# OpenMined/PIR

Hardware: AMD Instinct MI355X
Metric: PIR queries/sec (ms/query in ms_per_step), N=4096 DB=2^20 x 288B d=2 (higher is better)
Workload: dtype u64

## Files before the change

### pir_amd/csrc/ctx.hip

```cpp
#include <hip/hip_runtime.h>
#include <ctype.h>
#include <stdint.h>
#include <stdio.h>
#include <stdlib.h>
#include <string.h>

#include <algorithm>
#include <atomic>
#include <functional>
#include <map>
#include <mutex>
#include <string>
#include <vector>

#include "../../include/pirgpu.h"
#include "device_params.h"
#include "host_math.h"
#include "kernels.h"
#include "wire.h"

using namespace pirgpu;

namespace {

// ... 158 lines not shown
  uint64_t pt_words = 0;
  BatchSet sets[kBatchSets];
  BatchSet& bs();
  uint32_t n_active = 1;
  uint32_t upper_blocks = 512;
  uint32_t upper_blocks_batch = 64;
  uint32_t scan_wgs_batch = 128;
  bool in_batch = false;
  uint32_t scan_nsplit = 1, scan_cps = 0, scan_rows = 0, scan_cols = 0;
  uint32_t scan_rpt = 4, scan_block = 256;
  bool scan_limb = false;
  uint32_t mq_nq = 4, mq_rows = 1;
  bool mq_single = true;
  uint32_t mq_single_rows = 4;
  bool mq_single_limb = false;
  uint64_t scan_npt = 0;
  bool mfma_on = false;
  MfmaGeom mg{};
  uint32_t mfma_nq = kMaxMfmaQueries;
  bool mfma_single = true;
  bool scan_f64_fold = false;
  bool scan_f64_fold_batch = false;
  bool split_upper = false;
  uint64_t split_upper_words = (3ull << 30) / 8;
  bool loop_transforms = true;
  uint32_t loop_min_sources = 1024;
  uint32_t fuse_mac_nodes = 128;
  bool fuse_mac_combine = true;
  bool fuse_last_level = true;
  bool last_level_ntt = true;
  bool tree40 = true;
  bool c0_ntt = false;
  bool c0_ntt_split = false;
  bool want_sel_f64 = true;
  bool sel_f64 = false;
  bool pack40 = false;
  int pack_bytes = 5;
  uint8_t* d_dbp = nullptr;
  bool packed_valid = false;
  bool staging_released = false;
  std::vector<BatchLane> lanes;
  uint64_t groups_run = 0;
  hipStream_t head_stream = nullptr;
  uint32_t head_levels = 5;
  uint32_t head_mode = 1;
  hipEvent_t ev_head_tail = nullptr;
  hipStream_t copy_stream = nullptr;
  hipEvent_t ev_fetch[2] = {nullptr, nullptr};
  hipEvent_t ev_fork = nullptr;
  hipEvent_t ev_main_join = nullptr;

  bool prof = false;
  std::vector<hipEvent_t> bscan_ev;
  uint32_t bscan_n = 0, bscan_wgs = 0, bscan_nq = 0;
  static constexpr int kMaxProfRuns = 256;
  std::vector<hipEvent_t> ev;
  int prof_runs = 0;
  int prof_cur = -1;
  float timings[6]{};

  std::map<std::string, int64_t> opts;
  std::string err;
  uint64_t gen = 0;
  std::recursive_mutex mu;
  uint64_t zero_pts = 0;
  uint64_t remote_zero_pts = 0;
// ... 220 lines not shown
  }
  c->scan_npt = shard_pts;
  {
    auto env_u32 = [c](const char* name, uint32_t dflt) {
      return (uint32_t)option(c, name + 7, dflt);
    };
    c->scan_limb = true;
    for (uint32_t j = 0; j < k; ++j) c->scan_limb = c->scan_limb && (c->hp.mod[j].q >> 50) == 0;
    if (!env_u32("PIRGPU_SCAN_LIMB", 1)) c->scan_limb = false;
    c->mq_nq = 4;
    c->mq_rows = 1;
    c->mq_single = env_u32("PIRGPU_SCAN_MQ_SINGLE", 1) != 0;
    c->mq_single_rows = 4;
    c->mq_single_limb = false;
    c->scan_rpt = env_u32("PIRGPU_SCAN_ROWS", 4);
    c->scan_block = env_u32("PIRGPU_SCAN_BLOCK", 256);
    const uint32_t xblocks = (k * N / 2 + c->scan_block - 1) / c->scan_block;
    const uint32_t yblocks = (c->scan_rows + c->scan_rpt - 1) / c->scan_rpt;
    uint64_t have = (uint64_t)xblocks * std::max<uint32_t>(yblocks, 1) * c->scan_block / 256;
    uint32_t want = have >= 512 ? 1 : (uint32_t)ceil_div(1024, std::max<uint64_t>(have, 1));
    want = env_u32("PIRGPU_SCAN_NSPLIT", want);
    want = std::max<uint32_t>(1, std::min<uint32_t>(want, std::max<uint32_t>(c->scan_cols, 1)));
    c->scan_cps = (uint32_t)ceil_div(std::max<uint32_t>(c->scan_cols, 1), want);
    c->scan_nsplit = (uint32_t)ceil_div(std::max<uint32_t>(c->scan_cols, 1), c->scan_cps);
    c->fuse_last_level = env_u32("PIRGPU_FUSE_LAST", 1) != 0;
    c->fuse_mac_combine = env_u32("PIRGPU_FUSE_MAC_COMBINE", 1) != 0;
    c->last_level_ntt = env_u32("PIRGPU_LAST_NTT", 1) != 0;
    {
      const uint32_t v = env_u32("PIRGPU_C0_NTT", 0);
      c->c0_ntt = v != 0;
      c->c0_ntt_split = v >= 2;
    }
    c->want_sel_f64 = env_u32("PIRGPU_SEL_F64", 1) != 0;
    c->tree40 = env_u32("PIRGPU_TREE40", 1) != 0;
    c->fuse_mac_nodes = 128;
    c->head_levels = std::min<uint32_t>(env_u32("PIRGPU_HEAD_LEVELS", c->head_levels), 8);
    c->head_mode = std::min<uint32_t>(env_u32("PIRGPU_HEAD_MODE", c->head_mode), 2);
    c->split_upper = env_u32("PIRGPU_SPLIT_UPPER", c->logN >= 14 ? 1 : 0) != 0 && c->mode != kNttInt;
    c->split_upper_words = (uint64_t)env_u32("PIRGPU_SPLIT_UPPER_MB", 3072) * (1ull << 20) / 8;
    c->loop_transforms = env_u32("PIRGPU_LOOP_TRANSFORMS", 1) != 0 && c->mode != kNttInt;
    c->pack40 = env_u32("PIRGPU_PACK40", 1) != 0;
    {
      uint32_t bits = 0;
      for (uint32_t j = 0; j <= k; ++j) bits = std::max<uint32_t>(bits, 64 - (uint32_t)__builtin_clzll(c->hp.mod[j].q));
      const int need = bits <= 39 ? 5 : (bits <= 47 ? 6 : (bits <= 55 ? 7 : 8));
      int want = (int)env_u32("PIRGPU_PACK_BYTES", (uint32_t)need);
      if (want < need) want = need;
      if (c->mode == kNttInt && want != 5) want = 8;
      if (want > 7) c->pack40 = false;
      c->pack_bytes = c->pack40 ? want : 5;
      if (c->pack40 && c->pack_bytes == 7 && c->logN >= 14 && !env_u32("PIRGPU_TREE40_WIDE", 0)) c->tree40 = false;
      const NttOps* ops = ntt_ops_for(N, c->pack_bytes);
      if (ops != c->ops) {
        c->ops = ops;
        HIP_TRY(c->ops->configure(c->mode));
      }
    }
    bool wide_given = false;
    const int64_t wide = option(c, "SCAN_MFMA_WIDE", 0, &wide_given);
    c->mg = mfma_geometry(c->hp, c->scan_rows, c->scan_cols, wide_given ? (int)(wide != 0) : -1,
                          env_u32("PIRGPU_SCAN_MFMA_TOP4", 1) != 0);
    c->mfma_on = env_u32("PIRGPU_SCAN_MFMA", 1) != 0 && d >= 2 && c->mg.L != 0 && c->scan_rows >= 8 && shard_pts > 0;
    if (c->slot_sharded && (!c->mfma_on || c->mg.nchunks != 1 || c->nslots % c->mg.NW))
      throw Fail{PIRGPU_INVALID_ARGUMENT, "a slot shard needs the int8-MFMA scan in one column chunk (d = 2, >= 8 rows, "
                                          "moduli below 2^55, at most 28 column groups)"};
    c->mfma_nq = std::max<uint32_t>(1, std::min<uint32_t>(env_u32("PIRGPU_SCAN_MFMA_NQ", kMaxMfmaQueries),
// ... 140 lines not shown
  HIP_TRY(hipStreamSynchronize(st));
  c->gperm[g] = buf;
  return buf;
}

struct TreeState {
  uint64_t* cur = nullptr;
  bool cur40 = false;
  bool c0ntt = false;
};

uint64_t* expand_core(pirgpu_ctx* c, hipStream_t st, uint64_t* res_a, uint64_t* res_b, uint64_t* dig, uint64_t* prod,
                      uint32_t n, uint32_t B, const MfmaPtrs* sel_dst = nullptr, bool sel_f64 = false,
                      const uint32_t* ksets = nullptr, uint32_t j_begin = 0, uint32_t j_end = UINT32_MAX,
                      const TreeState* from = nullptr, TreeState* to = nullptr,
                      const std::function<void()>& after_first = nullptr) {
  const uint32_t N = c->N, k = c->k;
  if (n > N) throw Fail{PIRGPU_INVALID_ARGUMENT, "Cannot expand more items from a CT than poly modulus degree"};
  const uint32_t logm = hm::ceil_log2(n);
  const bool fuse_last = sel_dst && c->mode != kNttInt && c->fuse_last_level;
  if (sel_f64 && !(fuse_last && c->last_level_ntt && n >= 2)) throw Fail{PIRGPU_INTERNAL, "double-form selectors need the NTT-domain last level"};
  uint64_t *cur = res_a, *nxt = res_b;
  bool cur40 = false;
  bool c0ntt = false;
  if (from) {
    cur = from->cur;
    cur40 = from->cur40;
    c0ntt = from->c0ntt;
    nxt = res_a;
  }
  const uint32_t j_stop = std::min(j_end, logm);
  const bool c0_path = c->c0_ntt && fuse_last && c->last_level_ntt && c->mode != kNttInt && c->fuse_mac_combine;
  const uint32_t fuse_from = B > 1 ? std::max<uint32_t>(c->fuse_mac_nodes / 2, 1) : c->fuse_mac_nodes;
  auto level_fused = [&](uint32_t j) {
    return c->mode != kNttInt && c->fuse_mac_combine && ((1u << j) * B) >= fuse_from && !(fuse_last && j + 1 == logm);
  };
  for (uint32_t j = j_begin; j < j_stop; ++j) {
    auto level_done = [&]() {
      if (from && j == j_begin) {
        nxt = res_b;
        if (after_first) after_first();
      }
    };
    const uint32_t g = (N >> j) + 1;
    const KeyPtrs key = keys_for(c, g, ksets, B);
    const uint32_t nodes = (1u << j) * B;
    const bool last_ntt = fuse_last && j + 1 == logm && c->last_level_ntt;
    const bool c0_in_digit = last_ntt && !c0ntt && ks_digit_takes_c0(nodes);
    if (cur40 && !(last_ntt ? (c0ntt || c0_in_digit) : true)) throw Fail{PIRGPU_INTERNAL, "5-byte tree reached a level that cannot read it"};
    if (c0_path && !c0ntt && level_fused(j) && !cur40 && !(from && j == j_begin)) {
      HIP_TRY(c->ops->tree_c0_fwd(st, c->mode, c->dp, k, cur, nodes));
      c0ntt = true;
    }
    HIP_TRY(c->ops->ks_digit(st, c->mode, c->dp, k, cur, g, nodes, dig, c->pack40, c0_in_digit ? prod : nullptr, cur40,
                             c->loop_transforms && (uint64_t)nodes * k >= c->loop_min_sources));
    if (level_fused(j)) {
      const uint32_t next_nodes = nodes * 2;
      const bool next_last = j + 2 == logm;
      const bool next_reads40 = next_last ? (fuse_last && c->last_level_ntt && (c0ntt || ks_digit_takes_c0(next_nodes)))
                                          : (next_nodes >= fuse_from);
      const bool out40 = c->tree40 && c->pack40 && j + 1 < logm && next_reads40 && (1u << j) < (N >> ntt_log_ept((int)c->logN));
      HIP_TRY(c->ops->ks_mac_intt(st, c->mode, c->dp, k, dig, key, nodes, prod, c->pack40, k, 1));
      HIP_TRY(c->ops->ks_mac_combine(st, c->mode, c->dp, k, dig, key, prod, cur, g, nodes, 1u << j, nxt, c->pack40, cur40,
                                     out40, c0ntt ? xpow_table(c, st, 1u << j) : nullptr,
                                     c0ntt ? galois_perm_table(c, st, g) : nullptr, c->c0_ntt_split));
      cur40 = out40;
      std::swap(cur, nxt);
      level_done();
      continue;
    }
    if (cur40 && !last_ntt) throw Fail{PIRGPU_INTERNAL, "5-byte tree reached an unfused level"};
    if (c0ntt && !last_ntt) throw Fail{PIRGPU_INTERNAL, "NTT-form c0 reached an unfused level"};
    if (fuse_last && j + 1 == logm && c->last_level_ntt) {
      const uint64_t* X = xpow_table(c, st, 1u << j);
      HIP_TRY(c->ops->ks_mac_intt(st, c->mode, c->dp, k, dig, key, nodes, prod, c->pack40, k, 1));
      HIP_TRY(c->ops->ks_last_ntt(st, c->mode, c->dp, k, cur, dig, key, prod, X, g, galois_inverse(g, N), 1u << j, n, B,
                                  *sel_dst, nodes, c->pack40, sel_f64, c0_in_digit, c0ntt ? (cur40 ? 2 : 1) : 0,
                                  galois_perm_table(c, st, g)));
      return nullptr;
    }
    HIP_TRY(c->ops->ks_mac_intt(st, c->mode, c->dp, k, dig, key, nodes, prod, c->pack40, 0, k + 1));
    if (fuse_last && j + 1 == logm) {
      HIP_TRY(c->ops->ks_last_level(st, c->mode, c->dp, k, cur, prod, g, 1u << j, n, B, *sel_dst, nodes, c->pack40));
      return nullptr;
    }
// ... 394 lines not shown
  delete c;
}

const char* pirgpu_last_error(const pirgpu_ctx* c) {
  if (!c) return "null context";
  if (t_last_error_ctx == c && t_last_error_gen == c->gen)
    return t_last_error.c_str();
  return c->err.c_str();
}

void pirgpu_set_error(pirgpu_ctx* c, const char* message) { (void)fail(c, 0, message ? message : ""); }

void pirgpu_request_lock(pirgpu_ctx* c) {
  if (c) c->mu.lock();
}
void pirgpu_request_unlock(pirgpu_ctx* c) {
  if (c) c->mu.unlock();
}

int pirgpu_set_transparent_policy(pirgpu_ctx* c, int allow) {
  return guarded(c, [&]() -> int {
    c->allow_transparent = allow != 0;
    return PIRGPU_OK;
  });
}

static const struct { const char* name; bool early; } kOptions[] = {
    {"UPPER_BLOCKS", true}, {"UPPER_BLOCKS_BATCH", true}, {"SCAN_MFMA_WGS_BATCH", false}, {"SCAN_LIMB", true},
    {"SCAN_MQ_SINGLE", true}, {"SCAN_ROWS", true}, {"SCAN_BLOCK", true}, {"SCAN_NSPLIT", true},
    {"FUSE_LAST", true}, {"FUSE_MAC_COMBINE", true}, {"LAST_NTT", true}, {"C0_NTT", true}, {"SEL_F64", true}, {"TREE40", true},
    {"SPLIT_UPPER", true}, {"SPLIT_UPPER_MB", true}, {"PACK40", true}, {"PACK_BYTES", true}, {"TREE40_WIDE", true},
    {"SCAN_MFMA", true}, {"SCAN_MFMA_WIDE", true}, {"SCAN_MFMA_TOP4", true}, {"SCAN_MFMA_NQ", true}, {"SCAN_MFMA_SINGLE", true},
    {"HEAD_LEVELS", true}, {"HEAD_MODE", true}, {"SCAN_F64_FOLD", true}, {"SCAN_F64_FOLD_BATCH", true}, {"LOOP_TRANSFORMS", true},
    {"SLOTS_SCAN_WGS", false}, {"SLOTS_GATHER_NTT", false}, {"SLOTS_SCAN_BLK_MAJOR", false},
};

int pirgpu_set_option(pirgpu_ctx* c, const char* name, int64_t value) {
  return guarded(c, [&]() -> int {
    if (!name) return fail(c, PIRGPU_INVALID_ARGUMENT, "null option name");
    std::string up(name);
    for (char& ch : up) ch = (char)toupper((unsigned char)ch);
    for (const auto& o : kOptions) {
      if (up != o.name) continue;
      if (o.early && c->ws_ready)
        return fail(c, PIRGPU_FAILED_PRECONDITION, "option " + up + " shapes the workspace: set it before the context is first used");
      c->opts[up] = value;
      if (up == "SCAN_MFMA_WGS_BATCH") c->scan_wgs_batch = (uint32_t)std::max<int64_t>(0, value);
      return PIRGPU_OK;
    }
    return fail(c, PIRGPU_INVALID_ARGUMENT, "unknown option " + up);
  });
}

int pirgpu_get_option(pirgpu_ctx* c, const char* name, int64_t* value) {
  return guarded(c, [&]() -> int {
    if (!name || !value) return fail(c, PIRGPU_INVALID_ARGUMENT, "null argument");
    std::string up(name);
    for (char& ch : up) ch = (char)toupper((unsigned char)ch);
    for (const auto& o : kOptions)
      if (up == o.name) {
        bool present = false;
        *value = option(c, o.name, -1, &present);
        return PIRGPU_OK;
      }
    return fail(c, PIRGPU_INVALID_ARGUMENT, "unknown option " + up);
  });
}
// ... 1713 lines not shown
```

### pir_amd/csrc/kernels.h

```cpp
#pragma once
#include <hip/hip_runtime.h>
#include <stdint.h>

#include "device_params.h"

namespace pirgpu {

constexpr int kMaxScanChunks = 16;
constexpr int kMaxMfmaQueries = 8;
constexpr int kMaxScanGroups = 16;
constexpr int kMaxSlices = 16;

constexpr uint32_t kKsWideLevel = 256;
inline bool ks_digit_takes_c0(uint32_t nodes) { return nodes >= kKsWideLevel && nodes % 8 == 0; }

struct MfmaPtrs {
  const void* p[kMaxMfmaQueries];
};

struct ScanGroups {
  uint32_t n;
  const uint8_t* sel[kMaxScanGroups];
  uint64_t* out[kMaxScanGroups];
  uint8_t nq[kMaxScanGroups];
// ... 24 lines not shown
  hipError_t (*ks_digit)(hipStream_t st, int mode, const DevParams* P, uint32_t k, const uint64_t* res_in,
                         uint32_t galois_elt, uint32_t nodes, uint64_t* dig, bool pack40, uint64_t* c0_out, bool tree40,
                         bool loop_targets);
  hipError_t (*ks_mac_intt)(hipStream_t st, int mode, const DevParams* P, uint32_t k, const uint64_t* dig,
                            const KeyPtrs& key, uint32_t nodes, uint64_t* prod, bool pack40, uint32_t I_base,
                            uint32_t I_count);
  hipError_t (*upper_fused)(hipStream_t st, int mode, const DevParams* P, uint32_t k, uint32_t enc_count,
                            const uint64_t* src, const MfmaPtrs& svq, uint64_t* part, uint32_t n_rows,
                            uint32_t n_dim, uint32_t n_children_total, uint32_t sv_first, uint32_t C,
                            uint32_t chunk_len, uint32_t n_chunks, uint32_t n_queries, uint64_t src_qstride,
                            uint64_t part_qstride, bool sel_f64);
  hipError_t (*ks_last_level)(hipStream_t st, int mode, const DevParams* P, uint32_t k, const uint64_t* tree,
                              const uint64_t* prod, uint32_t galois_elt, uint32_t shift_pow, uint32_t n_items,
                              uint32_t B, const MfmaPtrs& dst, uint32_t tree_cts, bool pack40);
  hipError_t (*upper_ntt)(hipStream_t st, int mode, const DevParams* P, uint32_t k, uint32_t enc_count,
                          const uint64_t* src, uint64_t* scratch, uint32_t n_rows, uint32_t n_dim,
                          uint32_t n_children_total, uint32_t C, uint32_t b0, uint32_t blk, uint32_t n_queries,
                          uint64_t src_qstride, bool loop_source);
  hipError_t (*ks_mac_combine)(hipStream_t st, int mode, const DevParams* P, uint32_t k, const uint64_t* dig,
                               const KeyPtrs& key, const uint64_t* prod, const uint64_t* tree_in, uint32_t galois_elt,
                               uint32_t nodes, uint32_t shift_pow, uint64_t* tree_out, bool pack40, bool tin40,
                               bool tout40, const uint64_t* xpow_c0ntt,
                               const uint16_t* perm,
                               bool c0_split);
  hipError_t (*ks_last_ntt)(hipStream_t st, int mode, const DevParams* P, uint32_t k, const uint64_t* tree,
                            const uint64_t* dig, const KeyPtrs& key, uint64_t* prod, const uint64_t* xpow,
                            uint32_t galois_elt, uint32_t galois_inv, uint32_t shift_pow, uint32_t n_items, uint32_t B,
                            const MfmaPtrs& dst, uint32_t nodes, bool pack40, bool out_f64, bool c0_done, int c0_tree,
                            const uint16_t* perm);
  hipError_t (*ntt_inv_gather)(hipStream_t st, int mode, const DevParams* P, uint32_t k, const uint64_t* src,
                               uint64_t* dst, const SliceMap& map, uint32_t RC, uint32_t nq, uint32_t nq_total,
                               uint32_t q0);
  hipError_t (*tree_c0_fwd)(hipStream_t st, int mode, const DevParams* P, uint32_t k, uint64_t* tree, uint32_t cts);
};

const NttOps* ntt_ops_for(uint32_t N, int pack_bytes = 5);

hipError_t launch_ntt_reorder(hipStream_t st, uint32_t N, const uint64_t* in, uint64_t* out, uint64_t n_polys,
                              bool to_device, bool as_f64);
hipError_t launch_pack40x4(hipStream_t st, const uint64_t* in, uint32_t* out, uint64_t words);
hipError_t launch_unpack40x4(hipStream_t st, const uint32_t* in, uint64_t* out, uint64_t words);
hipError_t launch_ks_combine(hipStream_t st, const DevParams* P, int mode, uint32_t N, uint32_t k,
                             const uint64_t* res_in, const uint64_t* prod, uint32_t galois_inv, uint32_t nodes,
                             uint32_t shift_pow, bool expand_step, uint32_t hi_limit, bool pack40, uint64_t* res_out,
                             int pack_bytes = 5);
hipError_t launch_tree_convert(hipStream_t st, const DevParams* P, int mode, const uint64_t* in, uint64_t* out,
                               uint64_t words, bool to_tree, uint64_t chunk_words = 0, uint64_t in_stride = 0);
hipError_t launch_monomial_shift(hipStream_t st, const DevParams* P, uint32_t N, uint32_t k, const uint64_t* in,
                                 uint32_t shift, uint64_t count, uint64_t* out);
hipError_t launch_scan(hipStream_t st, const DevParams* P, uint32_t N, uint32_t k, const uint64_t* db,
                       const uint64_t* sv, uint64_t* out, uint32_t rows, uint32_t cols, uint64_t num_pt,
                       uint32_t nsplit, uint32_t cols_per_split, uint32_t rows_per_thread, uint32_t block,
                       bool limb);
hipError_t launch_scan_mq(hipStream_t st, const DevParams* P, uint32_t N, uint32_t k, const uint64_t* db,
                          const uint64_t* const* sv, uint64_t* const* out, uint32_t nq, uint32_t rows,
                          uint32_t cols, uint32_t rows_per_wave, bool limb);
hipError_t launch_reduce_splits(hipStream_t st, const DevParams* P, const uint64_t* part, uint32_t nsplit,
                                uint64_t words, uint64_t* out, uint32_t n_queries = 1, uint64_t part_qstride = 0,
                                uint64_t out_qstride = 0);


hipError_t launch_upper_mac(hipStream_t st, const DevParams* P, const uint64_t* scratch, const MfmaPtrs& svq,
                            uint64_t* acc, uint64_t* out, uint32_t n_queries, uint32_t n_rows, uint32_t C,
                            uint32_t enc_count, uint32_t k, uint32_t N, uint32_t sv_first, uint32_t b0, uint32_t blk,
                            uint32_t n_dim, bool first, bool last, uint64_t acc_qstride, uint64_t out_qstride);

// ... 32 lines not shown
```

### pir_amd/csrc/ntt_kernels.hip

```cpp
#include <hip/hip_runtime.h>
#include <stdint.h>
#include <stdlib.h>

#include "device_params.h"
#include "kernels.h"
#include "ntt_core.h"

#ifndef PIRGPU_LOGN
#error "compile with -DPIRGPU_LOGN=<11..14>"
#endif

#ifndef PIRGPU_PACK_BYTES
#define PIRGPU_PACK_BYTES 5
#endif
#define PIRGPU_CAT2(a, b) a##b
#define PIRGPU_CAT(a, b) PIRGPU_CAT2(a, b)
#if PIRGPU_PACK_BYTES == 5
#define PIRGPU_OPS_NAME PIRGPU_CAT(ntt_ops_, PIRGPU_LOGN)
#define PIRGPU_DEG_NS PIRGPU_CAT(deg, PIRGPU_LOGN)
#else
#define PIRGPU_OPS_NAME PIRGPU_CAT(PIRGPU_CAT(ntt_ops_, PIRGPU_LOGN), PIRGPU_CAT(_p, PIRGPU_PACK_BYTES))
#define PIRGPU_DEG_NS PIRGPU_CAT(PIRGPU_CAT(deg, PIRGPU_LOGN), PIRGPU_CAT(p, PIRGPU_PACK_BYTES))
#endif

// ... 683 lines not shown
    for (int e = 0; e < EPT; ++e) tlo[e * NT + tid_e] = t[e];
  }
  uint32_t tid_x = tid_e;
  asm volatile("" : "+v"(tid_x) : : "memory");
#pragma unroll
  for (int e = 0; e < EPT; ++e) t[e] = f64_mulmod(f64_norm(v[e] - x[e], m), X[e * NT + tid_x], m);
  if constexpr (TOUT40) {
    store40f(reinterpret_cast<uint8_t*>(tree_out_raw) + phi * kPoly40, tid_x, t, magic);
  } else {
    double* thi = reinterpret_cast<double*>(tree_out_raw) + phi * N;
#pragma unroll
    for (int e = 0; e < EPT; ++e) thi[e * NT + tid_x] = t[e];
  }
}

template <int MODE, bool P40, bool TIN40, bool TOUT40>
__global__ void __launch_bounds__(NT)
ks_c0_ntt_kernel(const DevParams* __restrict__ P, const uint64_t* __restrict__ dig_raw, KeyPtrs keys,
                 const uint64_t* __restrict__ prod, const uint64_t* __restrict__ tree_in_raw, uint32_t galois_elt,
                 uint32_t nodes, uint64_t* __restrict__ tree_out_raw, const double* __restrict__ xpow,
                 const uint16_t* __restrict__ perm) {
  static_assert(MODE != kNttInt, "fp64 flavours only");
  const uint32_t k = P->k;
  uint32_t node = blockIdx.x, j = blockIdx.y;
  if (gridDim.y == 1) {
    const uint32_t xcd = blockIdx.x & 7, t = blockIdx.x >> 3;
    j = t % k;
    node = (t / k) * 8 + xcd;
  }
  ks_combine_c0_ntt<MODE, P40, TIN40, TOUT40>(P, dig_raw, keys.p[node % keys.B], prod, tree_in_raw, xpow, perm, galois_elt, nodes,
                                              node, j, threadIdx.x, tree_out_raw);
}

template <int MODE, bool P40, bool TIN40 = false, bool TOUT40 = false, bool C0NTT = false>
__global__ void __launch_bounds__(NT) PIRGPU_MC_WAVES PIRGPU_PK_WAVES
ks_mac_combine_kernel(const DevParams* __restrict__ P, const uint64_t* __restrict__ dig_raw,
                      KeyPtrs keys, const uint64_t* __restrict__ prod,
                      const uint64_t* __restrict__ tree_in_raw, uint32_t galois_elt, uint32_t nodes, uint32_t shift_pow,
                      uint64_t* __restrict__ tree_out_raw, const double* __restrict__ xpow,
                      const uint16_t* __restrict__ perm, uint32_t comp1_only) {
  using A = Arith<MODE>;
  static_assert(MODE != kNttInt, "fp64 flavours only");
  double* sd = reinterpret_cast<double*>(smem_raw);
  const uint32_t tid = threadIdx.x, k = P->k, km = k + 1;
  uint32_t node = blockIdx.x, j = blockIdx.y, comp = blockIdx.z;
  if (gridDim.y == 1 && gridDim.z == 1) {
    const uint32_t xcd = blockIdx.x & 7, t = blockIdx.x >> 3;
    comp = comp1_only ? 1 : t & 1;
    const uint32_t u = comp1_only ? t : t >> 1;
    j = u % k;
    node = (u / k) * 8 + xcd;
  } else if (comp1_only) {
    comp = 1;
  }
  if constexpr (C0NTT) {
    if (comp == 0) {
      ks_combine_c0_ntt<MODE, P40, TIN40, TOUT40>(P, dig_raw, keys.p[node % keys.B], prod, tree_in_raw, xpow, perm, galois_elt,
                                                  nodes, node, j, tid, tree_out_raw);
      return;
    }
  }
  const typename A::Mod m = A::mod(P, j);
  double g[EPT];
  ks_mac_core<MODE, P40>(P, dig_raw, keys.p[node % keys.B], node, j, comp, tid, g);
  {
    const double pf = P->p_f, half = P->p_half_f, pinv = P->p_inv_f[j];
// ... 1 lines not shown
    [[maybe_unused]] Hi16 hs{};
    if constexpr (P40) hs = load40f_hi(reinterpret_cast<const uint8_t*>(prod) + spoly * kPoly40, tid);
#pragma unroll
    for (int e = 0; e < EPT; ++e) {
      double sp;
      if constexpr (P40) {
        sp = load40f(reinterpret_cast<const uint8_t*>(prod) + spoly * kPoly40, hs, e, tid, f64_pack_magic(pf));
      } else {
        sp = reinterpret_cast<const double*>(prod)[spoly * N + e * NT + tid];
      }
      sp = sp > half ? sp - pf : sp;
      sp = sp < -half ? sp + pf : sp;
      g[e] = f64_mulmod(g[e] - f64_norm(sp, m), pinv, m);
    }
  }
  if (!C0NTT && comp == 0) {
    const uint32_t raw0 = tid * galois_elt, rstep = (uint32_t)NT * galois_elt;
    double c0[EPT];
    tree_load<TIN40>(tree_in_raw, (size_t)node * 2 * k + j, tid, m.q, c0);
    __syncthreads();
#pragma unroll
    for (int e = 0; e < EPT; ++e) {
      const uint32_t raw = raw0 + (uint32_t)e * rstep;
      const uint64_t sign = (uint64_t)((raw << (31 - LOGN)) & 0x80000000u) << 32;
      sd[lds_idx<R_>(raw & (N - 1))] = __longlong_as_double((long long)((uint64_t)__double_as_longlong(c0[e]) ^ sign));
    }
    __syncthreads();
#pragma unroll
    for (int e = 0; e < EPT; ++e) g[e] += sd[lds_lin_base<NT, R_>(tid) + lds_lin_off<NT, R_>(e)];
  }
  const size_t opoly = (size_t)comp * k + j;
  double a[EPT];
  tree_load<TIN40>(tree_in_raw, (size_t)node * 2 * k + opoly, tid, m.q, a);
  if constexpr (TOUT40) {
    const double magic = f64_pack_magic(m.q);
    uint8_t* plo = reinterpret_cast<uint8_t*>(tree_out_raw) + ((size_t)node * 2 * k + opoly) * kPoly40;
    uint8_t* phi = reinterpret_cast<uint8_t*>(tree_out_raw) + (((size_t)node + nodes) * 2 * k + opoly) * kPoly40;
    double lo[EPT];
#pragma unroll
    for (int e = 0; e < EPT; ++e) lo[e] = f64_norm(a[e] + g[e], m);
    store40f(plo, tid, lo, magic);
    const bool borrow = tid < shift_pow;
    const uint32_t tid_d = (tid - shift_pow) & (NT - 1);
    uint32_t hb[EPT];
#pragma unroll
    for (int e = 0; e < EPT; ++e) {
      double d = f64_norm(a[e] - g[e], m);
      if (e == 0) d = borrow ? -d : d;
      uint32_t l32;
      f64_pack40(d, magic, l32, hb[e]);
      reinterpret_cast<uint32_t*>(phi)[(e * NT + tid - shift_pow) & (N - 1)] = l32;
    }
    uint32_t w[kHW];
    pack_hi_bytes(hb, w);
    uint32_t o[kHW];
#pragma unroll
    for (int q4 = 0; q4 < kHW; ++q4)
      o[q4] = borrow ? __builtin_amdgcn_alignbyte(w[(q4 + 1) % kHW], w[q4], kHB) : w[q4];
    store_hi_words(phi, tid_d, o);
  } else {
    const size_t off = opoly * N;
    double* tree_lo = reinterpret_cast<double*>(tree_out_raw) + (size_t)node * 2 * k * N + off;
    double* tree_hi = reinterpret_cast<double*>(tree_out_raw) + ((size_t)node + nodes) * 2 * k * N + off;
#pragma unroll
    for (int e = 0; e < EPT; ++e) {
      const uint32_t i = e * NT + tid;
      tree_lo[i] = f64_norm(a[e] + g[e], m);
      const double d = f64_norm(a[e] - g[e], m);
      const uint32_t sraw = i + (2 * N - shift_pow);
      tree_hi[sraw & (N - 1)] = (sraw & N) ? -d : d;
    }
  }
}

template <int MODE, bool P40>
__global__ void __launch_bounds__(NT)
ks_last_level_kernel(const DevParams* __restrict__ P, const uint64_t* __restrict__ tree_raw,
                     const uint64_t* __restrict__ prod, uint32_t galois_elt, uint32_t shift_pow, uint32_t n_items,
                     uint32_t B, MfmaPtrs dst) {
  using A = Arith<MODE>;
  static_assert(MODE != kNttInt, "fp64 flavours only");
  double* sd = reinterpret_cast<double*>(smem_raw);
  const uint32_t tid = threadIdx.x, k = P->k, km = k + 1;
  const uint32_t half_id = blockIdx.x & 1, bx = blockIdx.x >> 1;
  const uint32_t j = bx % k, comp = (bx / k) & 1, ct = bx / (2 * k);
  const uint32_t slot = ct / B, q = ct % B;
  const uint32_t out_slot = half_id ? slot + shift_pow : slot;
  if (out_slot >= n_items) return;
  const typename A::Mod m = A::mod(P, j);
  const double pf = P->p_f, half = P->p_half_f, pinv = P->p_inv_f[j];
  const double* tree = reinterpret_cast<const double*>(tree_raw) + (size_t)ct * 2 * k * N;
  double g[EPT];
  [[maybe_unused]] Hi16 hs{}, hj{};
  if constexpr (P40) {
    const uint8_t* pr = reinterpret_cast<const uint8_t*>(prod) + ((size_t)ct * 2 + comp) * km * kPoly40;
    hs = load40f_hi(pr + (size_t)k * kPoly40, tid);
    hj = load40f_hi(pr + (size_t)j * kPoly40, tid);
  }
#pragma unroll
  for (int e = 0; e < EPT; ++e) {
    [[maybe_unused]] const uint32_t i = e * NT + tid;
    double sp, dj;
    if constexpr (P40) {
// ... 524 lines not shown
    PIRGPU_SET((ks_mac_combine_kernel<MODE, true, true, true>));
    PIRGPU_SET((ks_mac_combine_kernel<MODE, false, false, false, true>));
    PIRGPU_SET((ks_mac_combine_kernel<MODE, true, false, false, true>));
    PIRGPU_SET((ks_mac_combine_kernel<MODE, true, false, true, true>));
    PIRGPU_SET((ks_mac_combine_kernel<MODE, true, true, false, true>));
    PIRGPU_SET((ks_mac_combine_kernel<MODE, true, true, true, true>));
    PIRGPU_SET(tree_c0_fwd_kernel<MODE>);
    PIRGPU_SET((ks_c0_ntt_kernel<MODE, false, false, false>));
    PIRGPU_SET((ks_c0_ntt_kernel<MODE, true, false, false>));
    PIRGPU_SET((ks_c0_ntt_kernel<MODE, true, false, true>));
    PIRGPU_SET((ks_c0_ntt_kernel<MODE, true, true, false>));
    PIRGPU_SET((ks_c0_ntt_kernel<MODE, true, true, true>));
    PIRGPU_SET((ks_digit_kernel<MODE, true, true>));
    PIRGPU_SET((ks_digit_kernel<MODE, false, false, true>));
    PIRGPU_SET((ks_digit_kernel<MODE, true, false, true>));
    PIRGPU_SET((ks_digit_kernel<MODE, true, true, true>));
    PIRGPU_SET((upper_ntt_kernel<MODE, true>));
    PIRGPU_SET((ks_last_level_kernel<MODE, false>));
    PIRGPU_SET((ks_last_level_kernel<MODE, true>));
    PIRGPU_SET((tree_c0_ntt_kernel<MODE, false>));
    PIRGPU_SET((tree_c0_ntt_kernel<MODE, true>));
    PIRGPU_SET((ks_last_ntt_kernel<MODE, false>));
    PIRGPU_SET((ks_last_ntt_kernel<MODE, true>));
    PIRGPU_SET((ks_last_ntt_kernel<MODE, false, true>));
    PIRGPU_SET((ks_last_ntt_kernel<MODE, true, true>));
    PIRGPU_SET((ks_last_ntt_kernel<MODE, false, false, 1>));
    PIRGPU_SET((ks_last_ntt_kernel<MODE, false, true, 1>));
    PIRGPU_SET((ks_last_ntt_kernel<MODE, true, false, 1>));
    PIRGPU_SET((ks_last_ntt_kernel<MODE, true, true, 1>));
    PIRGPU_SET((ks_last_ntt_kernel<MODE, true, false, 2>));
    PIRGPU_SET((ks_last_ntt_kernel<MODE, true, true, 2>));
    PIRGPU_SET((upper_fused_kernel<MODE, false, true>));
  }
#undef PIRGPU_SET
  return hipSuccess;
}

static hipError_t op_configure(int mode) {
  PIRGPU_BY_MODE(mode, return configure_mode<MODE>());
  return hipSuccess;
}

static hipError_t op_ntt_batch(hipStream_t st, int mode, const DevParams* P, uint64_t* data, uint64_t n_polys,
                               uint32_t mod_period, uint32_t mod_base, bool inverse) {
  if (inverse) {
    PIRGPU_BY_MODE(mode, hipLaunchKernelGGL((ntt_batch_kernel<MODE, true>), dim3((uint32_t)n_polys), dim3(NT),
                                            kLdsBytes, st, P, data, mod_period, mod_base));
  } else {
    PIRGPU_BY_MODE(mode, hipLaunchKernelGGL((ntt_batch_kernel<MODE, false>), dim3((uint32_t)n_polys), dim3(NT),
                                            kLdsBytes, st, P, data, mod_period, mod_base));
  }
  return hipGetLastError();
}

static hipError_t op_ntt_inv_gather(hipStream_t st, int mode, const DevParams* P, uint32_t k, const uint64_t* src,
                                    uint64_t* dst, const SliceMap& map, uint32_t RC, uint32_t nq, uint32_t nq_total,
                                    uint32_t q0) {
  if (map.n == 0 || map.n > (uint32_t)kMaxSlices || map.cut[0] != 0 || map.cut[map.n] != k * (uint32_t)N || q0 + nq > nq_total)
    return hipErrorInvalidValue;
  for (uint32_t r = 0; r <= map.n; ++r)
    if (map.cut[r] % NT) return hipErrorInvalidValue;
  PIRGPU_BY_MODE(mode, hipLaunchKernelGGL(ntt_inv_gather_kernel<MODE>, dim3(nq * RC * k), dim3(NT), kLdsBytes, st, P, src, dst,
                                          map, RC, nq_total, q0));
  return hipGetLastError();
}

// ... 242 lines not shown
    return hipErrorInvalidValue;
  return hipGetLastError();
}

static hipError_t op_upper_fused(hipStream_t st, int mode, const DevParams* P, uint32_t k, uint32_t enc_count,
                                 const uint64_t* src, const MfmaPtrs& svq, uint64_t* part, uint32_t n_rows,
                                 uint32_t n_dim, uint32_t n_children_total, uint32_t sv_first, uint32_t C,
                                 uint32_t chunk_len, uint32_t n_chunks, uint32_t n_queries, uint64_t src_qstride,
                                 uint64_t part_qstride, bool sel_f64) {
  const dim3 grid(n_queries * n_rows * C * n_chunks, enc_count, k);
#define PIRGPU_UF_ARGS P, src, svq, part, n_rows, n_dim, n_children_total, sv_first, C, chunk_len, n_chunks, src_qstride, part_qstride
  if (sel_f64 && mode == kNttInt) return hipErrorInvalidValue;
  if constexpr (kUpperLdsTw) {
    static const bool lds_tw = pirgpu_env("PIRGPU_UPPER_LDS_TW") && atoi(pirgpu_env("PIRGPU_UPPER_LDS_TW")) != 0;
    if (lds_tw && mode != kNttInt) {
      const size_t lds = kLdsBytes + (size_t)N * 8;
      if (mode == kNttF64 && sel_f64) hipLaunchKernelGGL((upper_fused_kernel<kNttF64, true, true>), grid, dim3(NT), lds, st, PIRGPU_UF_ARGS);
      else if (mode == kNttF64) hipLaunchKernelGGL((upper_fused_kernel<kNttF64, true>), grid, dim3(NT), lds, st, PIRGPU_UF_ARGS);
      else if (sel_f64) hipLaunchKernelGGL((upper_fused_kernel<kNttF64Wide, true, true>), grid, dim3(NT), lds, st, PIRGPU_UF_ARGS);
      else hipLaunchKernelGGL((upper_fused_kernel<kNttF64Wide, true>), grid, dim3(NT), lds, st, PIRGPU_UF_ARGS);
      return hipGetLastError();
    }
  }
  if (sel_f64) {
    if (mode == kNttF64) hipLaunchKernelGGL((upper_fused_kernel<kNttF64, false, true>), grid, dim3(NT), kLdsBytes, st, PIRGPU_UF_ARGS);
    else hipLaunchKernelGGL((upper_fused_kernel<kNttF64Wide, false, true>), grid, dim3(NT), kLdsBytes, st, PIRGPU_UF_ARGS);
    return hipGetLastError();
  }
  PIRGPU_BY_MODE(mode, hipLaunchKernelGGL(upper_fused_kernel<MODE>, grid, dim3(NT), kLdsBytes, st, PIRGPU_UF_ARGS));
#undef PIRGPU_UF_ARGS
  return hipGetLastError();
}

}

const NttOps* PIRGPU_OPS_NAME() {
  using namespace PIRGPU_DEG_NS;
  static const NttOps ops = {op_configure, op_ntt_batch,   op_ct_ntt_fwd_oop, op_ct_ntt_fwd_split, op_db_encode,
                             op_ks_digit,  op_ks_mac_intt, op_upper_fused,     op_ks_last_level,
                             op_upper_ntt, op_ks_mac_combine, op_ks_last_ntt, op_ntt_inv_gather, op_tree_c0_fwd};
  return &ops;
}

}
```

Measured before the change: 5556.

## Fuse key-switch digit, MAC/iNTT and tree combine into one per-node kernel

Adds a single kernel that handles one expansion-tree level per node for N=4096, k=2, 5-byte packing. It does the Galois automorphism, forward NTT of the digits, key multiply-accumulate, inverse NTT with mod-switch and the tree combine all within one workgroup of (k+1)*NT threads, keeping intermediates in LDS. This replaces three launches and their global round-trips through the digit and product buffers. The cost is heavy LDS use per block, which lowers occupancy, and more serialized work per block.

```diff
diff --git a/pir_amd/csrc/ctx.hip b/pir_amd/csrc/ctx.hip
--- a/pir_amd/csrc/ctx.hip
+++ b/pir_amd/csrc/ctx.hip
@@ -214,6 +214,7 @@
   bool tree40 = true;
   bool c0_ntt = false;
   bool c0_ntt_split = false;
+  bool ks_fused = true;
   bool want_sel_f64 = true;
   bool sel_f64 = false;
   bool pack40 = false;
@@ -500,6 +501,7 @@
       c->c0_ntt_split = v >= 2;
     }
     c->want_sel_f64 = env_u32("PIRGPU_SEL_F64", 1) != 0;
+    c->ks_fused = env_u32("PIRGPU_KS_FUSED", 1) != 0;
     c->tree40 = env_u32("PIRGPU_TREE40", 1) != 0;
     c->fuse_mac_nodes = 128;
     c->head_levels = std::min<uint32_t>(env_u32("PIRGPU_HEAD_LEVELS", c->head_levels), 8);
@@ -706,9 +708,12 @@
   const uint32_t j_stop = std::min(j_end, logm);
   const bool c0_path = c->c0_ntt && fuse_last && c->last_level_ntt && c->mode != kNttInt && c->fuse_mac_combine;
   const uint32_t fuse_from = B > 1 ? std::max<uint32_t>(c->fuse_mac_nodes / 2, 1) : c->fuse_mac_nodes;
+  const bool fused_kernel = c->ks_fused && c->ops->ks_fused && c->mode == kNttF64 && k == 2 && c->pack40 &&
+                            c->pack_bytes == 5 && !c0_path;
   auto level_fused = [&](uint32_t j) {
     return c->mode != kNttInt && c->fuse_mac_combine && ((1u << j) * B) >= fuse_from && !(fuse_last && j + 1 == logm);
   };
+  auto uses_fused_kernel = [&](uint32_t j) { return fused_kernel && B > 1 && level_fused(j); };
   for (uint32_t j = j_begin; j < j_stop; ++j) {
     auto level_done = [&]() {
       if (from && j == j_begin) {
@@ -725,6 +730,17 @@
     if (c0_path && !c0ntt && level_fused(j) && !cur40 && !(from && j == j_begin)) {
       HIP_TRY(c->ops->tree_c0_fwd(st, c->mode, c->dp, k, cur, nodes));
       c0ntt = true;
+    }
+    if (uses_fused_kernel(j)) {
+      const bool next_last = j + 2 == logm;
+      const bool next_reads40 = next_last ? (fuse_last && c->last_level_ntt && ks_digit_takes_c0(nodes * 2))
+                                          : level_fused(j + 1);
+      const bool out40 = c->tree40 && c->pack40 && j + 1 < logm && next_reads40 && (1u << j) < (N >> ntt_log_ept((int)c->logN));
+      HIP_TRY(c->ops->ks_fused(st, c->mode, c->dp, k, key, cur, g, nodes, 1u << j, nxt, cur40, out40));
+      cur40 = out40;
+      std::swap(cur, nxt);
+      level_done();
+      continue;
     }
     HIP_TRY(c->ops->ks_digit(st, c->mode, c->dp, k, cur, g, nodes, dig, c->pack40, c0_in_digit ? prod : nullptr, cur40,
                              c->loop_transforms && (uint64_t)nodes * k >= c->loop_min_sources));
@@ -1185,7 +1201,7 @@
     {"SPLIT_UPPER", true}, {"SPLIT_UPPER_MB", true}, {"PACK40", true}, {"PACK_BYTES", true}, {"TREE40_WIDE", true},
     {"SCAN_MFMA", true}, {"SCAN_MFMA_WIDE", true}, {"SCAN_MFMA_TOP4", true}, {"SCAN_MFMA_NQ", true}, {"SCAN_MFMA_SINGLE", true},
     {"HEAD_LEVELS", true}, {"HEAD_MODE", true}, {"SCAN_F64_FOLD", true}, {"SCAN_F64_FOLD_BATCH", true}, {"LOOP_TRANSFORMS", true},
-    {"SLOTS_SCAN_WGS", false}, {"SLOTS_GATHER_NTT", false}, {"SLOTS_SCAN_BLK_MAJOR", false},
+    {"KS_FUSED", true}, {"SLOTS_SCAN_WGS", false}, {"SLOTS_GATHER_NTT", false}, {"SLOTS_SCAN_BLK_MAJOR", false},
 };
 
 int pirgpu_set_option(pirgpu_ctx* c, const char* name, int64_t value) {
diff --git a/pir_amd/csrc/kernels.h b/pir_amd/csrc/kernels.h
--- a/pir_amd/csrc/kernels.h
+++ b/pir_amd/csrc/kernels.h
@@ -80,6 +80,9 @@
                                uint64_t* dst, const SliceMap& map, uint32_t RC, uint32_t nq, uint32_t nq_total,
                                uint32_t q0);
   hipError_t (*tree_c0_fwd)(hipStream_t st, int mode, const DevParams* P, uint32_t k, uint64_t* tree, uint32_t cts);
+  hipError_t (*ks_fused)(hipStream_t st, int mode, const DevParams* P, uint32_t k, const KeyPtrs& key,
+                         const uint64_t* tree_in, uint32_t galois_elt, uint32_t nodes, uint32_t shift_pow,
+                         uint64_t* tree_out, bool tin40, bool tout40);
 };
 
 const NttOps* ntt_ops_for(uint32_t N, int pack_bytes = 5);
diff --git a/pir_amd/csrc/ntt_kernels.hip b/pir_amd/csrc/ntt_kernels.hip
--- a/pir_amd/csrc/ntt_kernels.hip
+++ b/pir_amd/csrc/ntt_kernels.hip
@@ -739,6 +739,51 @@
                                               node, j, threadIdx.x, tree_out_raw);
 }
 
+template <bool TOUT40>
+__device__ __forceinline__ void ks_tree_store(uint64_t* __restrict__ tree_out_raw, uint32_t node, uint32_t nodes, uint32_t k,
+                                              size_t opoly, uint32_t shift_pow, const double (&a)[EPT],
+                                              const double (&g)[EPT], const F64Mod& m, uint32_t tid) {
+  if constexpr (TOUT40) {
+    const double magic = f64_pack_magic(m.q);
+    uint8_t* plo = reinterpret_cast<uint8_t*>(tree_out_raw) + ((size_t)node * 2 * k + opoly) * kPoly40;
+    uint8_t* phi = reinterpret_cast<uint8_t*>(tree_out_raw) + (((size_t)node + nodes) * 2 * k + opoly) * kPoly40;
+    double lo[EPT];
+#pragma unroll
+    for (int e = 0; e < EPT; ++e) lo[e] = f64_norm(a[e] + g[e], m);
+    store40f(plo, tid, lo, magic);
+    const bool borrow = tid < shift_pow;
+    const uint32_t tid_d = (tid - shift_pow) & (NT - 1);
+    uint32_t hb[EPT];
+#pragma unroll
+    for (int e = 0; e < EPT; ++e) {
+      double d = f64_norm(a[e] - g[e], m);
+      if (e == 0) d = borrow ? -d : d;
+      uint32_t l32;
+      f64_pack40(d, magic, l32, hb[e]);
+      reinterpret_cast<uint32_t*>(phi)[(e * NT + tid - shift_pow) & (N - 1)] = l32;
+    }
+    uint32_t w[kHW];
+    pack_hi_bytes(hb, w);
+    uint32_t o[kHW];
+#pragma unroll
+    for (int q4 = 0; q4 < kHW; ++q4)
+      o[q4] = borrow ? __builtin_amdgcn_alignbyte(w[(q4 + 1) % kHW], w[q4], kHB) : w[q4];
+    store_hi_words(phi, tid_d, o);
+  } else {
+    const size_t off = opoly * N;
+    double* tree_lo = reinterpret_cast<double*>(tree_out_raw) + (size_t)node * 2 * k * N + off;
+    double* tree_hi = reinterpret_cast<double*>(tree_out_raw) + ((size_t)node + nodes) * 2 * k * N + off;
+#pragma unroll
+    for (int e = 0; e < EPT; ++e) {
+      const uint32_t i = e * NT + tid;
+      tree_lo[i] = f64_norm(a[e] + g[e], m);
+      const double d = f64_norm(a[e] - g[e], m);
+      const uint32_t sraw = i + (2 * N - shift_pow);
+      tree_hi[sraw & (N - 1)] = (sraw & N) ? -d : d;
+    }
+  }
+}
+
 template <int MODE, bool P40, bool TIN40 = false, bool TOUT40 = false, bool C0NTT = false>
 __global__ void __launch_bounds__(NT) PIRGPU_MC_WAVES PIRGPU_PK_WAVES
 ks_mac_combine_kernel(const DevParams* __restrict__ P, const uint64_t* __restrict__ dig_raw,
@@ -806,43 +851,140 @@
   const size_t opoly = (size_t)comp * k + j;
   double a[EPT];
   tree_load<TIN40>(tree_in_raw, (size_t)node * 2 * k + opoly, tid, m.q, a);
-  if constexpr (TOUT40) {
-    const double magic = f64_pack_magic(m.q);
-    uint8_t* plo = reinterpret_cast<uint8_t*>(tree_out_raw) + ((size_t)node * 2 * k + opoly) * kPoly40;
-    uint8_t* phi = reinterpret_cast<uint8_t*>(tree_out_raw) + (((size_t)node + nodes) * 2 * k + opoly) * kPoly40;
-    double lo[EPT];
-#pragma unroll
-    for (int e = 0; e < EPT; ++e) lo[e] = f64_norm(a[e] + g[e], m);
-    store40f(plo, tid, lo, magic);
-    const bool borrow = tid < shift_pow;
-    const uint32_t tid_d = (tid - shift_pow) & (NT - 1);
-    uint32_t hb[EPT];
+  ks_tree_store<TOUT40>(tree_out_raw, node, nodes, k, opoly, shift_pow, a, g, m, tid);
+}
+
+constexpr bool kFusedLevel = LOGN == 12 && kPB == 5;
+constexpr uint32_t kFusedK = 2;
+constexpr int kFusedNT = (int)(kFusedK + 1) * NT;
+constexpr size_t kFusedStash = (size_t)(kFusedK + 1) * Plan<LOGN>::LDS_WORDS * 8;
+constexpr size_t kFusedLdsBytes = kFusedStash + (size_t)(kFusedK + 1) * N * 4;
+
+template <bool TIN40, bool TOUT40>
+__global__ void __launch_bounds__(kFusedNT)
+ks_fused_kernel(const DevParams* __restrict__ P, KeyPtrs keys, const uint64_t* __restrict__ tree_in_raw,
+                uint32_t galois_elt, uint32_t nodes, uint32_t shift_pow, uint64_t* __restrict__ tree_out_raw) {
+  using A = Arith<kNttF64>;
+  constexpr uint32_t k = kFusedK, km = k + 1;
+  const uint32_t I = __builtin_amdgcn_readfirstlane(threadIdx.x / NT), tid = threadIdx.x % NT;
+  const bool special = I == k;
+  double* sd = reinterpret_cast<double*>(smem_raw) + (size_t)I * Plan<LOGN>::LDS_WORDS;
+  const double* sp_lds = reinterpret_cast<const double*>(smem_raw) + (size_t)k * Plan<LOGN>::LDS_WORDS;
+  uint32_t* stash = reinterpret_cast<uint32_t*>(smem_raw + kFusedStash) + (size_t)I * N;
+  const uint32_t node = blockIdx.x;
+  const double* key = reinterpret_cast<const double*>(keys.p[node % keys.B]);
+  const typename A::Mod m = A::mod(P, I);
+  const double magic = f64_pack_magic(m.q);
+  double d0[EPT], x[EPT];
+#pragma clang loop unroll(disable)
+  for (uint32_t J = 0; J < k; ++J) {
+    uint32_t tl = tid;
+    asm volatile("" : "+v"(tl));
+    const double qJd = P->tab[J].qd;
+    const uint32_t raw0 = tl * galois_elt, rstep = (uint32_t)NT * galois_elt;
+    double c1[EPT];
+    tree_load<TIN40>(tree_in_raw, ((size_t)node * 2 + 1) * k + J, tl, qJd, c1);
+    __syncthreads();
 #pragma unroll
     for (int e = 0; e < EPT; ++e) {
-      double d = f64_norm(a[e] - g[e], m);
-      if (e == 0) d = borrow ? -d : d;
-      uint32_t l32;
-      f64_pack40(d, magic, l32, hb[e]);
-      reinterpret_cast<uint32_t*>(phi)[(e * NT + tid - shift_pow) & (N - 1)] = l32;
-    }
-    uint32_t w[kHW];
-    pack_hi_bytes(hb, w);
-    uint32_t o[kHW];
-#pragma unroll
-    for (int q4 = 0; q4 < kHW; ++q4)
-      o[q4] = borrow ? __builtin_amdgcn_alignbyte(w[(q4 + 1) % kHW], w[q4], kHB) : w[q4];
-    store_hi_words(phi, tid_d, o);
-  } else {
-    const size_t off = opoly * N;
-    double* tree_lo = reinterpret_cast<double*>(tree_out_raw) + (size_t)node * 2 * k * N + off;
-    double* tree_hi = reinterpret_cast<double*>(tree_out_raw) + ((size_t)node + nodes) * 2 * k * N + off;
-#pragma unroll
-    for (int e = 0; e < EPT; ++e) {
-      const uint32_t i = e * NT + tid;
-      tree_lo[i] = f64_norm(a[e] + g[e], m);
-      const double d = f64_norm(a[e] - g[e], m);
-      const uint32_t sraw = i + (2 * N - shift_pow);
-      tree_hi[sraw & (N - 1)] = (sraw & N) ? -d : d;
+      const uint32_t raw = raw0 + (uint32_t)e * rstep;
+      const uint64_t sign = (uint64_t)((raw << (31 - LOGN)) & 0x80000000u) << 32;
+      double v = __longlong_as_double((long long)((uint64_t)__double_as_longlong(c1[e]) ^ sign));
+      v = v < 0.0 ? v + qJd : v;
+      sd[lds_idx<R_>(raw & (N - 1))] = v;
+    }
+    __syncthreads();
+#pragma unroll
+    for (int e = 0; e < EPT; ++e) x[e] = sd[lds_lin_base<NT, R_>(tl) + lds_lin_off<NT, R_>(e)];
+    __syncthreads();
+    ntt_forward<kNttF64, LOGN, false, false>(x, sd, P, I, tl);
+    if (J == 0) {
+#pragma unroll
+      for (int e = 0; e < EPT; ++e) d0[e] = x[e];
+    }
+  }
+  Hi16 hi0;
+  {
+    uint32_t hb0[EPT];
+    uint32_t tl = tid;
+    asm volatile("" : "+v"(tl));
+    const uint64_t* key64 = reinterpret_cast<const uint64_t*>(key);
+    const __amdgpu_buffer_rsrc_t r00 = poly_rsrc(key64 + ((size_t)(0 * 2 + 0) * km + I) * N);
+    const __amdgpu_buffer_rsrc_t r01 = poly_rsrc(key64 + ((size_t)(0 * 2 + 1) * km + I) * N);
+    const __amdgpu_buffer_rsrc_t r10 = poly_rsrc(key64 + ((size_t)(1 * 2 + 0) * km + I) * N);
+    const __amdgpu_buffer_rsrc_t r11 = poly_rsrc(key64 + ((size_t)(1 * 2 + 1) * km + I) * N);
+    auto kw = [&](__amdgpu_buffer_rsrc_t r, int e) { return __longlong_as_double((long long)poly_load_u64(r, tl, e)); };
+#pragma unroll
+    for (int e4 = 0; e4 < EPT; e4 += 4) {
+#pragma unroll
+      for (int e = e4; e < e4 + 4; ++e) {
+        double s0 = 0.0, s1 = 0.0;
+        s0 += f64_mulmod(d0[e], kw(r00, e), m);
+        s1 += f64_mulmod(d0[e], kw(r01, e), m);
+        s0 += f64_mulmod(x[e], kw(r10, e), m);
+        s1 += f64_mulmod(x[e], kw(r11, e), m);
+        uint32_t lo;
+        f64_pack40(f64_norm(s0, m), magic, lo, hb0[e]);
+        stash[e * NT + tl] = lo;
+        x[e] = f64_norm(s1, m);
+      }
+      asm volatile("" : "+v"(tl) : "v"(x[e4 + 3]));
+    }
+    pack_hi_bytes(hb0, hi0.w);
+  }
+  const double pf = P->p_f, half = P->p_half_f;
+  const double pinv = special ? 0.0 : P->p_inv_f[I];
+#pragma clang loop unroll(disable)
+  for (uint32_t comp = 1; comp < 2; --comp) {
+    uint32_t tl = tid;
+    asm volatile("" : "+v"(tl));
+    if (comp == 0) {
+      __syncthreads();
+#pragma unroll
+      for (int e = 0; e < EPT; ++e) {
+        const uint32_t lo = stash[e * NT + tl];
+        x[e] = __longlong_as_double((long long)(((uint64_t)hi_word(hi0, e) << 32) | lo)) - magic;
+      }
+    }
+    ntt_inverse<kNttF64, LOGN, false, false>(x, sd, P, I, tl);
+    __syncthreads();
+    if (special) {
+#pragma unroll
+      for (int e = 0; e < EPT; ++e) sd[e * NT + tl] = x[e];
+    }
+    __syncthreads();
+    if (!special) {
+#pragma unroll
+      for (int e = 0; e < EPT; ++e) {
+        double sp = sp_lds[e * NT + tl];
+        sp = sp > half ? sp - pf : sp;
+        sp = sp < -half ? sp + pf : sp;
+        x[e] = f64_mulmod(x[e] - f64_norm(sp, m), pinv, m);
+      }
+    }
+    if (comp == 0) {
+      if (!special) {
+        const uint32_t raw0 = tl * galois_elt, rstep = (uint32_t)NT * galois_elt;
+        double c0[EPT];
+        tree_load<TIN40>(tree_in_raw, (size_t)node * 2 * k + I, tl, m.q, c0);
+#pragma unroll
+        for (int e = 0; e < EPT; ++e) {
+          const uint32_t raw = raw0 + (uint32_t)e * rstep;
+          const uint64_t sign = (uint64_t)((raw << (31 - LOGN)) & 0x80000000u) << 32;
+          sd[lds_idx<R_>(raw & (N - 1))] = __longlong_as_double((long long)((uint64_t)__double_as_longlong(c0[e]) ^ sign));
+        }
+      }
+      __syncthreads();
+      if (!special) {
+#pragma unroll
+        for (int e = 0; e < EPT; ++e) x[e] += sd[lds_lin_base<NT, R_>(tl) + lds_lin_off<NT, R_>(e)];
+      }
+    }
+    if (!special) {
+      const size_t opoly = (size_t)comp * k + I;
+      double a[EPT];
+      tree_load<TIN40>(tree_in_raw, (size_t)node * 2 * k + opoly, tl, m.q, a);
+      ks_tree_store<TOUT40>(tree_out_raw, node, nodes, k, opoly, shift_pow, a, x, m, tl);
     }
   }
 }
@@ -1433,6 +1575,11 @@
     PIRGPU_SET((ks_last_ntt_kernel<MODE, true, true, 2>));
     PIRGPU_SET((upper_fused_kernel<MODE, false, true>));
   }
+  if constexpr (MODE == kNttF64 && kFusedLevel) {
+    for (const void* f : {(const void*)ks_fused_kernel<false, false>, (const void*)ks_fused_kernel<false, true>,
+                          (const void*)ks_fused_kernel<true, false>, (const void*)ks_fused_kernel<true, true>})
+      if ((e = hipFuncSetAttribute(f, hipFuncAttributeMaxDynamicSharedMemorySize, (int)kFusedLdsBytes))) return e;
+  }
 #undef PIRGPU_SET
   return hipSuccess;
 }
@@ -1741,13 +1888,33 @@
   return hipGetLastError();
 }
 
+static hipError_t op_ks_fused(hipStream_t st, int mode, const DevParams* P, uint32_t k, const KeyPtrs& key,
+                               const uint64_t* tree_in, uint32_t galois_elt, uint32_t nodes, uint32_t shift_pow,
+                               uint64_t* tree_out, bool tin40, bool tout40) {
+  if (mode != kNttF64 || k != kFusedK) return hipErrorInvalidValue;
+  if (tout40 && shift_pow >= (uint32_t)NT) return hipErrorInvalidValue;
+  if constexpr (kFusedLevel) {
+#define PIRGPU_FK(TI, TO)                                                                                         \
+  hipLaunchKernelGGL((ks_fused_kernel<TI, TO>), dim3(nodes), dim3(kFusedNT), kFusedLdsBytes, st, P, key, tree_in, \
+                     galois_elt, nodes, shift_pow, tree_out)
+    if (tin40 && tout40) PIRGPU_FK(true, true);
+    else if (tin40) PIRGPU_FK(true, false);
+    else if (tout40) PIRGPU_FK(false, true);
+    else PIRGPU_FK(false, false);
+#undef PIRGPU_FK
+    return hipGetLastError();
+  }
+  return hipErrorInvalidValue;
+}
+
 }
 
 const NttOps* PIRGPU_OPS_NAME() {
   using namespace PIRGPU_DEG_NS;
   static const NttOps ops = {op_configure, op_ntt_batch,   op_ct_ntt_fwd_oop, op_ct_ntt_fwd_split, op_db_encode,
                              op_ks_digit,  op_ks_mac_intt, op_upper_fused,     op_ks_last_level,
-                             op_upper_ntt, op_ks_mac_combine, op_ks_last_ntt, op_ntt_inv_gather, op_tree_c0_fwd};
+                             op_upper_ntt, op_ks_mac_combine, op_ks_last_ntt, op_ntt_inv_gather, op_tree_c0_fwd,
+                             kFusedLevel ? op_ks_fused : nullptr};
   return &ops;
 }
 
```

After: 5682, median of 6. 2.3% higher.
